# facebook/transform360

Measured on NVIDIA H100. Metric: Mpixels/s 8K equirect->cubemap bicubic (input-plane pixels consumed per second), higher is better.
Workload: dtype u8

## Files before the change

### profiles/trace_frame.py

```python
#!/usr/bin/env python
import sys
from pathlib import Path

import numpy as np
import torch

sys.path.insert(0, str(Path(__file__).resolve().parents[1]))
import transform360_b200 as t360
from bench import CONFIGS
from transform360_b200 import synth
from transform360_b200.stream import FrameTransformer, StreamSpec

KINDS = {0: "class0", 1: "class1", 3: "share-stay", 4: "share", 5: "nop", 7: "seam", 8: "pole-cap", 9: "border"}


def main():
    name = sys.argv[1] if len(sys.argv) > 1 else "cfg2"
    cfg = CONFIGS[name]
    dev = torch.device("cuda", 0)
    torch.cuda.set_device(0)
    ctx = t360.make_context(**dict(cfg["ov"], enable_low_pass_filter=0))
    spec = StreamSpec(cfg["inp"][0], cfg["inp"][1], cfg["out"][0], cfg["out"][1])
    ft = FrameTransformer(ctx, spec)
    pitch = lambda w: (w + 255) // 256 * 256
    ring = 5
    d_in = [[synth.noise_plane_torch(*spec.plane_dims(p)[:2], plane=p, frame=f, device=dev, pitch=pitch(spec.plane_dims(p)[0])) for p in range(3)]
            for f in range(ring)]
    d_out = [torch.zeros((spec.plane_dims(p)[3], pitch(spec.plane_dims(p)[2])), dtype=torch.uint8, device=dev) for p in range(3)]
    calls = [ft.frame_call([(t.data_ptr(), t.stride(0)) for t in fr], [(t.data_ptr(), t.stride(0)) for t in d_out]) for fr in d_in]
    stream = torch.cuda.Stream(device=dev)
    torch.cuda.synchronize()
    for i in range(6):
        calls[i % ring](stream.cuda_stream)
    torch.cuda.synchronize()
    ft.vft.debug_trace(True)
    calls[1](stream.cuda_stream)
    torch.cuda.synchronize()
    tr = ft.vft.read_trace().astype(np.int64)
    ft.vft.debug_trace(False)
    if len(sys.argv) > 2:
        np.save(sys.argv[2], tr)
    used = tr[..., 2] > 0
    t_start = tr[..., 0][used].min()
    end = np.where(used, tr[..., 2], 0).max(axis=1) - t_start
    begin = np.where(used, tr[..., 0], 1 << 62).min(axis=1) - t_start
    print(f"groups {tr.shape[0]}, jobs traced {int(used.sum())}, frame {end.max() / 1e3:.1f} us; groups finish at "
          f"min {end.min() / 1e3:.1f} / median {np.median(end) / 1e3:.1f} / max {end.max() / 1e3:.1f} us, start at median {np.median(begin) / 1e3:.1f} us")
    wait, comp, kind = (tr[..., 1] - tr[..., 0])[used], (tr[..., 2] - tr[..., 1])[used], tr[..., 3][used]
    print(f"all jobs: waiting {wait.sum() / 1e3:.0f} group-us, computing {comp.sum() / 1e3:.0f} group-us "
          f"({100 * wait.sum() / (wait.sum() + comp.sum()):.0f} % waiting)")
    for k in sorted(set(kind.tolist())):
        m = kind == k
        print(f"  {KINDS.get(k, k):10s} n={int(m.sum()):5d}  wait mean {wait[m].mean():7.0f} ns (p90 {np.percentile(wait[m], 90):6.0f})  "
              f"compute mean {comp[m].mean():7.0f} ns (p10 {np.percentile(comp[m], 10):6.0f} p90 {np.percentile(comp[m], 90):6.0f})")
    first = tr[:, 0, :]
    print(f"first job of a group: wait {np.mean(first[:, 1] - first[:, 0]) / 1e3:.2f} us")


if __name__ == "__main__":
    main()
```

### transform360_b200/csrc/gather_frame.cu

```cuda
#include "gather_common.cuh"

#include <cuda.h>

#include <algorithm>
#include <cstring>
#include <utility>

namespace t360 {

namespace {

template <class F, int... I>
__device__ __forceinline__ void staticForImpl(F&& f, std::integer_sequence<int, I...>) {
  (f(std::integral_constant<int, I>{}), ...);
}
template <int N, class F>
__device__ __forceinline__ void staticFor(F&& f) {
  staticForImpl(f, std::make_integer_sequence<int, N>{});
}

template <int IMM>
__device__ __forceinline__ uint32_t ldsWordImm(uint32_t addr) {
  uint32_t v;
  asm volatile("ld.shared.u32 %0, [%1+%2];" : "=r"(v) : "r"(addr), "n"(IMM));
  return v;
}
template <int IMM>
__device__ __forceinline__ uint4 ldsVecImm(uint32_t addr) {
  uint4 v;
  asm volatile("ld.shared.v4.u32 {%0, %1, %2, %3}, [%4+%5];" : "=r"(v.x), "=r"(v.y), "=r"(v.z), "=r"(v.w) : "r"(addr), "n"(IMM));
  return v;
}
template <int IMM>
__device__ __forceinline__ uint2 ldsVec2Imm(uint32_t addr) {
  uint2 v;
  asm volatile("ld.shared.v2.u32 {%0, %1}, [%2+%3];" : "=r"(v.x), "=r"(v.y) : "r"(addr), "n"(IMM));
  return v;
}

__device__ __forceinline__ uint32_t smemAddr(const void* p) { return (uint32_t)__cvta_generic_to_shared(p); }

__device__ __forceinline__ void mbarInit(uint64_t* bar, uint32_t arrivals) {
  asm volatile("mbarrier.init.shared::cta.b64 [%0], %1;" ::"r"(smemAddr(bar)), "r"(arrivals));
}
__device__ __forceinline__ void mbarExpectTx(uint64_t* bar, uint32_t bytes) {
  asm volatile("mbarrier.arrive.expect_tx.shared::cta.b64 _, [%0], %1;" ::"r"(smemAddr(bar)), "r"(bytes) : "memory");
}
__device__ __forceinline__ void mbarWait(uint64_t* bar, uint32_t parity) {
  asm volatile(
      "{\n\t.reg .pred p;\n\t"
      "WAIT_%=:\n\t"
      "mbarrier.try_wait.parity.shared::cta.b64 p, [%0], %1;\n\t"
      "@p bra DONE_%=;\n\t"
      "bra WAIT_%=;\n\t"
      "DONE_%=:\n\t}"
      ::"r"(smemAddr(bar)), "r"(parity) : "memory");
}
__device__ __forceinline__ void tmaLoadBox(void* dst, const CUtensorMap* map, int x, int y, uint64_t* bar) {
  asm volatile(
      "cp.async.bulk.tensor.2d.shared::cluster.global.mbarrier::complete_tx::bytes [%0], [%1, {%2, %3}], [%4];"
      ::"r"(smemAddr(dst)), "l"(reinterpret_cast<uint64_t>(map)), "r"(x), "r"(y), "r"(smemAddr(bar)) : "memory");
}
__device__ __forceinline__ void bulkCopyToShared(void* dst, const void* src, uint32_t bytes, uint64_t* bar) {
  asm volatile("cp.async.bulk.shared::cluster.global.mbarrier::complete_tx::bytes [%0], [%1], %2, [%3];"
               ::"r"(smemAddr(dst)), "l"(src), "r"(bytes), "r"(smemAddr(bar)) : "memory");
}
__device__ __forceinline__ void groupBarrier(int group) {
  asm volatile("bar.sync %0, %1;" ::"r"(group + 1), "n"(kGroupThreads) : "memory");
}

template <int K>
struct RowBytes {
  uint32_t b[K == 8 ? 2 : 1];
};

template <int K, int IMM>
__device__ __forceinline__ RowBytes<K> loadRow(uint32_t addr, int sh) {
  RowBytes<K> o;
  const uint32_t q0 = ldsWordImm<IMM>(addr), q1 = ldsWordImm<IMM + 4>(addr);
  o.b[0] = __funnelshift_r(q0, q1, sh);
  if constexpr (K == 8) o.b[1] = __funnelshift_r(q1, ldsWordImm<IMM + 8>(addr), sh);
  return o;
}

template <int K, int VS>
__device__ __forceinline__ int foldRows(const RowBytes<K> (&W)[K], uint32_t slotAddr) {
  int acc = 1 << 14;
  if constexpr (K == 2) {
    const uint2 w = ldsVec2Imm<0>(slotAddr);
    acc = dp2aLo(w.x, W[0].b[0], acc);
    acc = dp2aLo(w.y, W[1].b[0], acc);
  } else if constexpr (K == 4) {
    const uint4 wa = ldsVecImm<0>(slotAddr), wb = ldsVecImm<VS>(slotAddr);
    acc = dp2aLo(wa.x, W[0].b[0], acc); acc = dp2aHi(wa.y, W[0].b[0], acc);
    acc = dp2aLo(wa.z, W[1].b[0], acc); acc = dp2aHi(wa.w, W[1].b[0], acc);
    acc = dp2aLo(wb.x, W[2].b[0], acc); acc = dp2aHi(wb.y, W[2].b[0], acc);
    acc = dp2aLo(wb.z, W[3].b[0], acc); acc = dp2aHi(wb.w, W[3].b[0], acc);
  } else {
    staticFor<8>([&](auto R) {
      constexpr int r = decltype(R)::value;
      const uint4 wt = ldsVecImm<r * VS>(slotAddr);
      acc = dp2aLo(wt.x, W[r].b[0], acc); acc = dp2aHi(wt.y, W[r].b[0], acc);
      acc = dp2aLo(wt.z, W[r].b[1], acc); acc = dp2aHi(wt.w, W[r].b[1], acc);
    });
  }
  return acc;
}
template <int K>
__device__ __forceinline__ uint32_t slotOffset(uint32_t field) { return K == 2 ? field >> 1 : field; }

template <int VS>
__device__ __forceinline__ int foldRowsRotated(const RowBytes<8> (&W)[8], uint32_t wAddr, uint32_t field) {
  static_assert(VS == 16384, "one copy of the table");
  const uint32_t r = ((field >> 4) ^ threadIdx.x) & 7u;
  const uint32_t first = field ^ (r * (uint32_t)kDiagonalStep);
  const bool p0 = (r & 1u) != 0, p1 = (r & 2u) != 0, p2 = (r & 4u) != 0;
  RowBytes<8> A[8], B[8];
#pragma unroll
  for (int i = 0; i < 8; ++i)
#pragma unroll
    for (int h = 0; h < 2; ++h) A[i].b[h] = p0 ? W[i ^ 1].b[h] : W[i].b[h];
#pragma unroll
  for (int i = 0; i < 8; ++i)
#pragma unroll
    for (int h = 0; h < 2; ++h) B[i].b[h] = p1 ? A[i ^ 2].b[h] : A[i].b[h];
  int acc = 1 << 14;
  staticFor<8>([&](auto V) {
    constexpr int v = decltype(V)::value;
    const uint4 wt = ldsVecImm<0>(wAddr + (first ^ (uint32_t)(v * kDiagonalStep)));
    const uint32_t b0 = p2 ? B[v ^ 4].b[0] : B[v].b[0], b1 = p2 ? B[v ^ 4].b[1] : B[v].b[1];
    acc = dp2aLo(wt.x, b0, acc); acc = dp2aHi(wt.y, b0, acc);
    acc = dp2aLo(wt.z, b1, acc); acc = dp2aHi(wt.w, b1, acc);
  });
  return acc;
}
template <int K, int VS>
__device__ __forceinline__ int foldPixel(const RowBytes<K> (&W)[K], uint32_t wAddr, uint32_t field) {
  if constexpr (K == 8) return foldRowsRotated<VS>(W, wAddr, field);
  else return foldRows<K, VS>(W, wAddr + slotOffset<K>(field));
}
__device__ __forceinline__ int biasedToByte(int acc) { return min(max(acc >> 15, 0), 255); }


__device__ __forceinline__ uint32_t packBytes(int hi, int lo) {
  uint32_t r;
  asm("cvt.pack.sat.u8.s32.b32 %0, %1, %2, %3;" : "=r"(r) : "r"(hi), "r"(lo), "r"(0));
  return r;
}

template <int K, int PITCH, int VS, int ROWS, bool ZERO>
__device__ __forceinline__ void computeShareJob(uint8_t* dst, int dstPitch, uint32_t stageAddr, const uint4 (&rec)[ROWS / 8],
                                                uint32_t header, uint32_t wAddr) {
  static_assert(PITCH % 4 == 0 && (K == 4 || K == 8) && ROWS % 8 == 0, "");
  uint32_t base = stageAddr + (header & 0x7ffcu);
  const int sh = (int)(header << 3);
  RowBytes<K> W[K];
  staticFor<K>([&](auto R) { W[decltype(R)::value] = loadRow<K, decltype(R)::value * PITCH>(base, sh); });
  int accPrev = 0;
  staticFor<ROWS>([&](auto J) {
    constexpr int j = decltype(J)::value;
    const uint4& block = rec[j >> 3];
    const uint32_t word = ((j >> 1) & 3) == 0 ? block.x : (((j >> 1) & 3) == 1 ? block.y : (((j >> 1) & 3) == 2 ? block.z : block.w));
    const uint32_t r = (j & 1) ? word >> 16 : word;
    if constexpr (j > 0 && !ZERO) {
      const bool two = (r & 1u) != 0;
      const RowBytes<K> below = loadRow<K, (j - 1 + K) * PITCH>(base, sh);
      RowBytes<K> below2 = below;
      if (two) below2 = loadRow<K, (j + K) * PITCH>(base, sh);
#pragma unroll
      for (int q = 0; q + 2 < K; ++q)
#pragma unroll
        for (int i = 0; i < (K == 8 ? 2 : 1); ++i) W[q].b[i] = two ? W[q + 2].b[i] : W[q + 1].b[i];
#pragma unroll
      for (int i = 0; i < (K == 8 ? 2 : 1); ++i) W[K - 2].b[i] = two ? below.b[i] : W[K - 1].b[i];
      W[K - 1] = below2;
      if (two) base += PITCH;
    }
    if constexpr (j > 0 && ZERO) {
      const uint32_t d = r & 3u;
      RowBytes<K> below = W[K - 1], below2 = W[K - 1];
      if (d != 0) below = loadRow<K, K * PITCH>(base, sh);
      if (d == 2) below2 = loadRow<K, (K + 1) * PITCH>(base, sh);
#pragma unroll
      for (int q = 0; q + 2 < K; ++q)
#pragma unroll
        for (int i = 0; i < (K == 8 ? 2 : 1); ++i) W[q].b[i] = d == 0 ? W[q].b[i] : (d == 1 ? W[q + 1].b[i] : W[q + 2].b[i]);
#pragma unroll
      for (int i = 0; i < (K == 8 ? 2 : 1); ++i) {
        W[K - 2].b[i] = d == 0 ? W[K - 2].b[i] : (d == 1 ? W[K - 1].b[i] : below.b[i]);
        W[K - 1].b[i] = d == 0 ? W[K - 1].b[i] : (d == 1 ? below.b[i] : below2.b[i]);
      }
      base += d * PITCH;
    }
    const int acc = foldPixel<K, VS>(W, wAddr, r & kSlotFieldMask) >> 15;
    if constexpr (j & 1) {
      const uint32_t pair = packBytes(acc, accPrev);
      dst[(size_t)(j - 1) * dstPitch] = (uint8_t)pair;
      dst[(size_t)j * dstPitch] = (uint8_t)(pair >> 8);
    } else {
      accPrev = acc;
    }
  });
}

template <int K, int PITCH, int VS>
__device__ __forceinline__ void computeTileJob(const PlaneView& pv, uint32_t stageAddr, int outX, int outY, const uint4& rec,
                                               uint32_t wAddr, int warp) {
  static_assert(PITCH % 4 == 0, "");
  const int y0 = outY + warp * kTilePatchH;
  const int dstPitch = pv.dstPitch, dstW = pv.dstW, dstH = pv.dstH;
  uint8_t* const dstRow = pv.dst + (size_t)y0 * dstPitch + outX;
  const uint32_t words[4] = {rec.x, rec.y, rec.z, rec.w};
  staticFor<kRowsPerPatchStep>([&](auto J) {
    constexpr int j = decltype(J)::value;
    const uint32_t w = words[j];
    const int col = kTilePatchW * j + ((int)(w >> 16) & (kTilePatchW - 1)), row = (int)(w >> 19) & (kTilePatchH - 1);
    if (!(w & kRecordSkip) && outX + col < dstW && y0 + row < dstH) {
      const uint32_t rowAddr = stageAddr + (w & 0x7ffcu);
      const int sh = (int)(w << 3);
      RowBytes<K> W[K];
      staticFor<K>([&](auto R) { W[decltype(R)::value] = loadRow<K, decltype(R)::value * PITCH>(rowAddr, sh); });
      const int acc = foldPixel<K, VS>(W, wAddr, (w >> 17) & kSlotFieldMask);
      dstRow[(size_t)row * dstPitch + col] = (uint8_t)biasedToByte(acc);
    }
  });
}

template <int K, int PITCH, int VS>
__device__ __forceinline__ void computeCapJob(const PlaneView& pv, uint32_t stageAddr, uint32_t recAddr, int steps, uint32_t wAddr,
                                              int warp, int lane) {
  static_assert(PITCH % 4 == 0, "");
  for (int s = warp; s < steps; s += kGroupWarps) {
    const uint2 r = ldsVec2Imm<0>(recAddr + s * kCapStepBytes + lane * 8);
    if (r.x & kRecordSkip) continue;
    const uint32_t rowAddr = stageAddr + (r.x & 0x7ffcu);
    const int sh = (int)(r.x << 3);
    RowBytes<K> W[K];
    staticFor<K>([&](auto R) { W[decltype(R)::value] = loadRow<K, decltype(R)::value * PITCH>(rowAddr, sh); });
    const int acc = foldPixel<K, VS>(W, wAddr, (r.x >> 17) & kSlotFieldMask);
    pv.dst[(size_t)(r.y >> 16) * pv.dstPitch + (r.y & 0xffffu)] = (uint8_t)biasedToByte(acc);
  }
}

template <int K, int VS>
__device__ __forceinline__ void computeBorderJob(const PlaneView& pv, uint32_t recAddr, int n, const unsigned char* wsmem, int warp, int lane) {
  SrcView sv;
  sv.bytes = pv.src;
  sv.misalign = (int)(reinterpret_cast<uintptr_t>(pv.src) & 3);
  sv.words = reinterpret_cast<const uint32_t*>(pv.src - sv.misalign);
  sv.w = pv.srcW; sv.h = pv.srcH; sv.pitch = pv.srcPitch;
  for (int i = warp * 32 + lane; i < n; i += kGroupThreads) {
    const uint4 r = ldsVecImm<0>(recAddr + i * kBorderPixelBytes);
    const int v = gatherPixel<K, false, VS, weightDiagonal(K)>(sv, wsmem, (int)r.x, (int)r.y);
    pv.dst[(size_t)(r.z >> 16) * pv.dstPitch + (r.z & 0xffffu)] = (uint8_t)v;
  }
}

struct FrameTensorMaps {
  CUtensorMap map[kMaxFramePlanes][kNumBoxClasses][kBoxVariants];
};

__device__ __forceinline__ void mbarArrive(uint64_t* bar) {
  asm volatile("mbarrier.arrive.shared::cta.b64 _, [%0];" ::"r"(smemAddr(bar)) : "memory");
}
__device__ __forceinline__ uint4 ldsVec(uint32_t addr) {
  uint4 v;
  asm volatile("ld.shared.v4.u32 {%0, %1, %2, %3}, [%4];" : "=r"(v.x), "=r"(v.y), "=r"(v.z), "=r"(v.w) : "r"(addr));
  return v;
}
__device__ __forceinline__ uint32_t ldsWord(uint32_t addr) {
  uint32_t v;
  asm volatile("ld.shared.u32 %0, [%1];" : "=r"(v) : "r"(addr));
  return v;
}

template <int K, int COPIES, int GROUPS>
struct FrameLayout {
  static constexpr int kStages = gatherStages(K);
  static constexpr int kWeights = weightImageBytes(K, COPIES);
  static constexpr int kStage = stageBytesOf(K), kRec = stageRecordBytes(K);
  static constexpr int kGroupBytes = kStages * (kStage + kRec);
  static constexpr int kPlanes = kWeights + GROUPS * kGroupBytes;
  static constexpr int kBars = kPlanes + 256;
  static constexpr int kTotal = kBars + GROUPS * kStages * 16 + 16;
  static_assert(kTotal <= 232448, "227 KB of shared memory per CTA");
  static_assert(sizeof(PlaneView) * kMaxFramePlanes <= 256, "");
  static_assert(kStage % 128 == 0 && kRec % 128 == 0 && kWeights % 128 == 0, "TMA / bulk-copy destinations");
};

template <int K, int COPIES, int GROUPS>
__global__ void __launch_bounds__(GROUPS * (kGroupWarps + 1) * 32, 1)
gatherFrameKernel(const __grid_constant__ FrameGatherParams p, StagedParams jobs, const __grid_constant__ FrameTensorMaps maps) {
  using L = FrameLayout<K, COPIES, GROUPS>;
  constexpr int VS = weightVectorStride(K, COPIES), kStage = L::kStage, kRec = L::kRec, S = L::kStages;
  constexpr uint32_t kBox0 = stageBoxW(K, 0) * stageBoxH(K, 0), kBox1 = stageBoxW(K, 1) * stageBoxH(K, 1),
                     kBoxShare = stageBoxW(K, 2) * stageBoxH(K, 2);
  static_assert(kBox1 + 64 <= 2 * kStage && kBox0 + 64 <= kStage && kBoxShare + 64 <= kStage, "boxes must fit their stage buffers");
  static_assert(boxVariantRows(K, 0, kBoxVariants - 1) > 0 && boxVariantRows(K, 2, kBoxVariants - 1) > 0, "");
  extern __shared__ __align__(128) unsigned char smem[];
  unsigned char* wsmem = smem;
  PlaneView* planes = reinterpret_cast<PlaneView*>(smem + L::kPlanes);
  uint64_t* barBase = reinterpret_cast<uint64_t*>(smem + L::kBars);
  uint64_t* weightBar = barBase + GROUPS * 2 * S;
  const int warpId = threadIdx.x >> 5, lane = threadIdx.x & 31;
  constexpr int kProducerWarp = GROUPS * kGroupWarps;

  asm volatile("griddepcontrol.launch_dependents;" ::: "memory");
  if (threadIdx.x == 0) {
    for (int g = 0; g < GROUPS; ++g)
      for (int st = 0; st < S; ++st) {
        mbarInit(barBase + g * 2 * S + st, 1);
        mbarInit(barBase + g * 2 * S + S + st, kGroupWarps);
      }
    mbarInit(weightBar, 1);
    asm volatile("fence.mbarrier_init.release.cluster;" ::: "memory");
  }
  if (threadIdx.x < kMaxFramePlanes * (int)(sizeof(PlaneView) / 4))
    reinterpret_cast<uint32_t*>(planes)[threadIdx.x] = reinterpret_cast<const uint32_t*>(p.plane)[threadIdx.x];
  __syncthreads();

  if (warpId >= kProducerWarp) {
    const int g = warpId - kProducerWarp;
    if (g == 0 && lane == 0) {
      mbarExpectTx(weightBar, L::kWeights);
      constexpr int kChunk = L::kWeights / 4;
      for (int i = 0; i < 4; ++i)
        bulkCopyToShared(wsmem + i * kChunk, reinterpret_cast<const unsigned char*>(p.weightImage) + i * kChunk, kChunk, weightBar);
    }
    const int producer = blockIdx.x * GROUPS + g, dynamicBase = gridDim.x * GROUPS * 2 * kClaimBatch;
    auto loadBatch = [&](int base) {
      int4 h = make_int4(0, kJobExit << kJobKindShift, 0, 0);
      if (lane < kClaimBatch && base + lane < jobs.numTiles) h = __ldg(reinterpret_cast<const int4*>(jobs.tiles) + base + lane);
      return h;
    };
    int4 batch = loadBatch(producer * 2 * kClaimBatch);
    int4 batchNext = loadBatch((producer * 2 + 1) * kClaimBatch);
    asm volatile("griddepcontrol.wait;" ::: "memory");
    int claimed = 0;
    if (lane == 0) claimed = atomicAdd(jobs.claimCounter, kClaimBatch);
    unsigned char* groupBase = smem + L::kWeights + g * L::kGroupBytes;
    uint64_t* full = barBase + g * 2 * S;
    uint64_t* empty = full + S;
    int pos = 0;
    uint32_t st = 0, phase = 0;
    auto advance = [&]() { if (++st == S) { st = 0; phase ^= 1; } };
    auto postEmptyJob = [&](int kind) {
      *reinterpret_cast<int4*>(groupBase + S * kStage + st * kRec) = make_int4(0, kind << kJobKindShift, 0, 0);
      mbarArrive(full + st);
    };
    for (;;) {
      if (pos == kClaimBatch) {
        batch = batchNext;
        pos = 0;
        batchNext = loadBatch(dynamicBase + __shfl_sync(0xffffffffu, claimed, 0));
        if (lane == 0) claimed = atomicAdd(jobs.claimCounter, kClaimBatch);
      }
      int4 h;
      h.x = __shfl_sync(0xffffffffu, batch.x, pos); h.y = __shfl_sync(0xffffffffu, batch.y, pos);
      h.z = __shfl_sync(0xffffffffu, batch.z, pos); h.w = __shfl_sync(0xffffffffu, batch.w, pos);
      ++pos;
      const int kind = (h.y >> kJobKindShift) & kJobKindMask;
      mbarWait(empty + st, phase ^ 1);
      const bool twoStages = kind == kJobClass1 || kind == kJobSeam;
      if (twoStages) {
        if (st == S - 1) {
          if (lane == 0) postEmptyJob(kJobNop);
          advance();
          mbarWait(empty + st, phase ^ 1);
        }
        mbarWait(empty + st + 1, phase ^ 1);
      }
      if (lane == 0) {
        unsigned char* rec = groupBase + S * kStage + st * kRec;
        *reinterpret_cast<int4*>(rec) = h;
        if (kind == kJobExit) {
          mbarArrive(full + st);
        } else {
          const int pl = h.y >> kJobPlaneShift;
          const uint32_t recBytes = (uint32_t)jobRecordBytes(K, kind, h.x);
          if (kind == kJobBorder) {
            mbarExpectTx(full + st, recBytes);
          } else {
            const int cls = boxClassOf(kind), variant = jobBoxVariant(h.z), boxX = jobBoxX(h.z), boxY = jobBoxY(h.z);
            const uint32_t boxBytes = (uint32_t)(stageBoxW(K, cls) * boxVariantRows(K, cls, variant));
            mbarExpectTx(full + st, (kind == kJobSeam ? 2 : 1) * boxBytes + recBytes);
            tmaLoadBox(groupBase + st * kStage, &maps.map[pl][cls][variant], boxX, boxY, full + st);
            if (kind == kJobSeam)
              tmaLoadBox(groupBase + (st + 1) * kStage, &maps.map[pl][0][variant], boxX - planes[pl].srcW, boxY, full + st);
          }
          bulkCopyToShared(rec + 128, planes[pl].records + (unsigned)h.w, recBytes, full + st);
        }
      }
      advance();
      if (twoStages) {
        if (lane == 0) postEmptyJob(kJobNop);
        advance();
      }
      __syncwarp();
      if (kind == kJobExit) break;
    }
    if (lane == 0 && atomicAdd(jobs.claimCounter + 1, 1) == (int)(gridDim.x * GROUPS) - 1) {
      jobs.claimCounter[0] = 0;
      jobs.claimCounter[1] = 0;
      __threadfence();
    }
    return;
  }

  const int group = warpId / kGroupWarps, warp = warpId % kGroupWarps;
  unsigned char* groupBase = smem + L::kWeights + group * L::kGroupBytes;
  const uint32_t boxAddr = smemAddr(groupBase), recAddr = smemAddr(groupBase + S * kStage);
  uint64_t* full = barBase + group * 2 * S;
  uint64_t* empty = full + S;
  const uint32_t wAddr = smemAddr(wsmem);
  mbarWait(weightBar, 0);
  asm volatile("griddepcontrol.wait;" ::: "memory");
  auto now = []() { unsigned long long t; asm volatile("mov.u64 %0, %globaltimer;" : "=l"(t)); return t; };
  unsigned long long* trace = jobs.trace && warp == 0 && lane == 0 ? jobs.trace + (size_t)(blockIdx.x * GROUPS + group) * kTraceJobsPerGroup * 4 : nullptr;
  uint32_t traced = 0;
  for (uint32_t st = 0, phase = 0;;) {
    unsigned long long* const row = trace && traced < kTraceJobsPerGroup ? trace + traced * 4 : nullptr;
    if (row) row[0] = now();
    mbarWait(full + st, phase);
    if (row) row[1] = now();
    const uint32_t rec = recAddr + st * kRec;
    const uint4 h = ldsVec(rec);
    const int kind = ((int)h.y >> kJobKindShift) & kJobKindMask;
    if (kind == kJobExit) break;
    const int outX = (int)h.x & ~kJobQuadMask, outY = (int)h.y & kJobRowMask;
    const PlaneView& pv = planes[(int)h.y >> kJobPlaneShift];
    if (kind == kJobShare || kind == kJobShareStay) {
      if constexpr (K >= 4) {
        const uint32_t mine = rec + 128 + warp * shareWarpRecordBytes(K);
        uint4 r[shareRows(K) / 8];
#pragma unroll
        for (int b = 0; b < shareRows(K) / 8; ++b) r[b] = ldsVec(mine + b * 512 + lane * 16);
        const uint32_t header = ldsWord(mine + shareRows(K) / 8 * 512 + lane * 4);
        uint8_t* dst = pv.dst + (size_t)(outY + (warp >> 1) * shareRows(K)) * pv.dstPitch + (outX + (warp & 1) * 32 + (int)(header >> kRecordColumnShift));
        if (kind == kJobShare) computeShareJob<K, stageBoxW(K, 2), VS, shareRows(K), false>(dst, pv.dstPitch, boxAddr + st * kStage, r, header, wAddr);
        else computeShareJob<K, stageBoxW(K, 2), VS, shareRows(K), true>(dst, pv.dstPitch, boxAddr + st * kStage, r, header, wAddr);
      }
    } else if (kind == kJobClass0) {
      uint4 r;
      const int quad = ((int)h.x & kJobQuadMask) - 1;
      if (quad < 0) {
        r = ldsVec(rec + 128 + warp * 512 + lane * 16);
      } else {
        r = make_uint4(kRecordSkip, kRecordSkip, kRecordSkip, kRecordSkip);
        if ((warp >> 2) == (quad >> 1)) {
          const uint2 v = ldsVec2Imm<0>(rec + 128 + (warp & 3) * 256 + lane * 8);
          if (quad & 1) { r.z = v.x; r.w = v.y; } else { r.x = v.x; r.y = v.y; }
        }
      }
      computeTileJob<K, stageBoxW(K, 0), VS>(pv, boxAddr + st * kStage, outX, outY, r, wAddr, warp);
    } else if (kind == kJobClass1) {
      computeTileJob<K, stageBoxW(K, 1), VS>(pv, boxAddr + st * kStage, outX, outY, ldsVec(rec + 128 + warp * 512 + lane * 16), wAddr, warp);
    } else if (kind == kJobSeam) {
      {
        uint4* a = reinterpret_cast<uint4*>(groupBase + st * kStage);
        const uint4* b = reinterpret_cast<const uint4*>(groupBase + (st + 1) * kStage);
        for (int i = warp * 32 + lane; i < (int)(kBox0 / 16); i += kGroupThreads) {
          uint4 x = a[i];
          const uint4 y = b[i];
          x.x |= y.x; x.y |= y.y; x.z |= y.z; x.w |= y.w;
          a[i] = x;
        }
        asm volatile("fence.proxy.async.shared::cta;" ::: "memory");
      }
      groupBarrier(group);
      computeTileJob<K, stageBoxW(K, 0), VS>(pv, boxAddr + st * kStage, outX, outY, ldsVec(rec + 128 + warp * 512 + lane * 16), wAddr, warp);
    } else if (kind == kJobCap) {
      computeCapJob<K, stageBoxW(K, 0), VS>(pv, boxAddr + st * kStage, rec + 128, (int)h.x, wAddr, warp, lane);
    } else if (kind == kJobBorder) {
      computeBorderJob<K, VS>(pv, rec + 128, (int)h.x, wsmem, warp, lane);
    }
    __syncwarp();
    if (lane == 0) mbarArrive(empty + st);
    if (row) {
      row[2] = now(); row[3] = kind;
      ++traced;
    }
    if (++st == S) { st = 0; phase ^= 1; }
  }
}

template <int K, int COPIES, int GROUPS>
cudaError_t prepareFrameK(LaunchCfg& cfg) {
  static DeviceLaunchCfg cfgs;
  constexpr int threads = GROUPS * (kGroupWarps + 1) * 32, smemBytes = FrameLayout<K, COPIES, GROUPS>::kTotal;
  return prepare<gatherFrameKernel<K, COPIES, GROUPS>>(cfgs, threads, smemBytes, cfg);
}

template <int K, int COPIES, int GROUPS>
cudaError_t launchFrameK(const FrameGatherParams& p, const StagedParams& jobs, const FrameTensorMaps& maps, int numSMs,
                         cudaStream_t stream, bool programmatic) {
  constexpr int threads = GROUPS * (kGroupWarps + 1) * 32, smemBytes = FrameLayout<K, COPIES, GROUPS>::kTotal;
  LaunchCfg cfg;
  cudaError_t err = prepareFrameK<K, COPIES, GROUPS>(cfg);
  if (err != cudaSuccess) return err;
  const int grid = std::min(numSMs * cfg.perSM, (jobs.numTiles + GROUPS * 2 * kClaimBatch - 1) / (GROUPS * 2 * kClaimBatch));
  cudaLaunchConfig_t lc{};
  lc.gridDim = dim3(grid);
  lc.blockDim = dim3(threads);
  lc.dynamicSmemBytes = smemBytes;
  lc.stream = stream;
  cudaLaunchAttribute attr{};
  attr.id = cudaLaunchAttributeProgrammaticStreamSerialization;
  attr.val.programmaticStreamSerializationAllowed = 1;
  lc.attrs = &attr;
  lc.numAttrs = programmatic ? 1 : 0;
  err = cudaLaunchKernelEx(&lc, gatherFrameKernel<K, COPIES, GROUPS>, p, jobs, maps);
  gLaunches.fetch_add(1, std::memory_order_relaxed);
  return err;
}

}

cudaError_t prepareGatherFrame(int kernelSize) {
  LaunchCfg cfg;
  switch (kernelSize) {
    case 2: return prepareFrameK<2, weightCopies(2), gatherGroups(2)>(cfg);
    case 4: return prepareFrameK<4, weightCopies(4), gatherGroups(4)>(cfg);
    case 8: return prepareFrameK<8, weightCopies(8), gatherGroups(8)>(cfg);
    default: return cudaErrorInvalidValue;
  }
}

cudaError_t launchGatherFrame(const FrameGatherParams& p, const StagedParams& jobs, const void* tensorMaps, int numSMs,
                              cudaStream_t stream, bool programmatic) {
  if (jobs.numTiles <= 0) return cudaSuccess;
  if (p.numPlanes < 1 || p.numPlanes > kMaxFramePlanes) return cudaErrorInvalidValue;
  FrameTensorMaps maps;
  std::memcpy(&maps, tensorMaps, sizeof(CUtensorMap) * kNumBoxClasses * kBoxVariants * p.numPlanes);
  for (int i = p.numPlanes; i < kMaxFramePlanes; ++i)
    for (int c = 0; c < kNumBoxClasses; ++c)
      for (int v = 0; v < kBoxVariants; ++v) maps.map[i][c][v] = maps.map[0][c][v];
  switch (p.kernelSize) {
    case 2: return launchFrameK<2, weightCopies(2), gatherGroups(2)>(p, jobs, maps, numSMs, stream, programmatic);
    case 4: return launchFrameK<4, weightCopies(4), gatherGroups(4)>(p, jobs, maps, numSMs, stream, programmatic);
    case 8: return launchFrameK<8, weightCopies(8), gatherGroups(8)>(p, jobs, maps, numSMs, stream, programmatic);
    default: return cudaErrorInvalidValue;
  }
}

}
```

### transform360_b200/csrc/kernels.cuh

```cuda
#pragma once

#include <cuda_runtime.h>

#include <cstdint>

namespace t360 {

struct GatherParams {
  const uint8_t* src;
  int srcW, srcH, srcPitch;
  uint8_t* dst;
  int dstW, dstH, dstPitch;
  const int2* samples;
  int tilesPerRow;
  const int16_t* weights;
  int kernelSize;
  int transparent;
};

struct GatherJob {
  int outX, outY;
  int boxXY;
  int recordOffset;
};
constexpr int kBoxVariants = 3;
__host__ __device__ constexpr int jobBoxField(int boxX, int boxY, int variant) { return boxX | (boxY << 16) | variant; }
__host__ __device__ constexpr int jobBoxX(int boxXY) { return boxXY & 0xfff0; }
__host__ __device__ constexpr int jobBoxY(int boxXY) { return (int)((unsigned)boxXY >> 16); }
__host__ __device__ constexpr int jobBoxVariant(int boxXY) { return boxXY & 15; }
using StagedTile = GatherJob;
constexpr int kJobClass0 = 0, kJobClass1 = 1, kJobGeneral = 2, kJobShareStay = 3, kJobShare = 4, kJobNop = 5, kJobExit = 6, kJobSeam = 7,
              kJobCap = 8, kJobBorder = 9;
constexpr int kJobQuadMask = 7;
constexpr uint32_t kRecordSkip = 0x8000u;
constexpr int kJobKindShift = 24, kJobRowMask = (1 << kJobKindShift) - 1;
constexpr int kJobPlaneShift = 28, kJobKindMask = (1 << (kJobPlaneShift - kJobKindShift)) - 1;

constexpr int kGroupThreads = 256, kGroupWarps = kGroupThreads / 32;
__host__ __device__ constexpr int gatherGroups(int k) { return k == 8 ? 2 : 3; }
#ifndef T360_CLAIM_BATCH
#define T360_CLAIM_BATCH 1
#endif
constexpr int kClaimBatch = T360_CLAIM_BATCH;
constexpr int kGatherTileW = 32, kFrameTileH = 32;
constexpr int kTilePatchW = 8, kTilePatchH = 4, kRowsPerPatchStep = 4;
constexpr int kShareW = 64;
__host__ __device__ constexpr int shareRows(int ) { return 8; }
__host__ __device__ constexpr int shareH(int k) { return 4 * shareRows(k); }
constexpr int kNumBoxClasses = 3;
__host__ __device__ constexpr int boxClassOf(int kind) { return (kind == kJobShare || kind == kJobShareStay) ? 2 : (kind == kJobClass1 ? 1 : 0); }
__host__ __device__ constexpr int stageBoxW(int , int cls) { return cls == 2 ? 192 : (cls == 0 ? 208 : 240); }
__host__ __device__ constexpr int stageBoxH(int k, int cls) {
  return k == 8 ? (cls == 2 ? 80 : (cls == 0 ? 72 : 128)) : (cls == 2 ? 72 : (cls == 0 ? 64 : 96));
}
__host__ __device__ constexpr int boxVariantRows(int k, int cls, int v) {
  return cls == 1 || v == 0 ? stageBoxH(k, cls) : (cls == 2 ? stageBoxH(k, cls) - 8 * v : stageBoxH(k, cls) - 8 - 8 * v);
}
__host__ __device__ constexpr int boxVariantFor(int k, int cls, int rows) {
  int v = 0;
  while (v + 1 < kBoxVariants && cls != 1 && boxVariantRows(k, cls, v + 1) >= rows) ++v;
  return v;
}
__host__ __device__ constexpr int gatherStages(int ) { return 2; }
__host__ __device__ constexpr int stageBytesOf(int k) {
  const int a = stageBoxW(k, 2) * stageBoxH(k, 2), b = stageBoxW(k, 0) * stageBoxH(k, 0);
  return ((a > b ? a : b) + 64 + 127) & ~127;
}

__host__ __device__ constexpr int weightSlotOf(int k, int phase) {
  (void)k;
  return (phase & ~31) | ((phase & 1) << 4) | ((phase & 31) >> 1);
}
__host__ __device__ constexpr int weightCopies(int k) { return k == 4 ? 2 : 1; }
__host__ __device__ constexpr int weightVectorStride(int k, int copies) { return (k == 2 ? 8192 : 16384) * copies; }
__host__ __device__ constexpr int weightImageBytes(int k, int copies) { return k == 2 ? 8192 * copies : (k * k / 8) * 16384 * copies; }
__host__ __device__ constexpr int weightSlotInCopy(int slot, int copy) { return copy ? ((slot & ~7) | ((slot + copy) & 7)) : slot; }
__host__ __device__ constexpr int weightSlotField(int k, int phase, int copy) {
  return (weightSlotInCopy(weightSlotOf(k, phase), copy) << 4) | (copy << 14);
}
constexpr int kSlotFieldMask = 0x7FF0;
constexpr int kDiagonalStep = 0x4010;
__host__ __device__ constexpr bool weightDiagonal(int k) { return k == 8; }
__host__ __device__ constexpr int weightVectorOffset(int k, int copies, int slotFieldValue, int vector) {
  return weightDiagonal(k) ? (slotFieldValue ^ (vector * kDiagonalStep)) : slotFieldValue + vector * weightVectorStride(k, copies);
}
__host__ __device__ constexpr int weightBankGroups(int k) { return k == 2 ? 16 : 8; }
__host__ __device__ constexpr int weightLanesPerPass(int k) { return k == 2 ? 16 : 8; }

__host__ __device__ constexpr int shareWarpRecordBytes(int k) { return shareRows(k) / 8 * 32 * 16 + 32 * 4; }
__host__ __device__ constexpr int shareJobRecordBytes(int k) { return kGroupWarps * shareWarpRecordBytes(k); }
constexpr int kTileJobRecordBytes = kGroupWarps * 32 * 16;
constexpr int kQuadJobRecordBytes = kGroupWarps / 2 * 32 * 8;
__host__ __device__ constexpr int tileJobRecordBytes(int outXField) { return (outXField & kJobQuadMask) ? kQuadJobRecordBytes : kTileJobRecordBytes; }
__host__ __device__ constexpr int stageRecordBytes(int k) {
  return 128 + (shareJobRecordBytes(k) > kTileJobRecordBytes ? shareJobRecordBytes(k) : kTileJobRecordBytes);
}
constexpr int kCapStepBytes = 32 * 8, kBorderPixelBytes = 16;
__host__ __device__ constexpr int capJobMaxSteps(int k) { return (stageRecordBytes(k) - 128) / kCapStepBytes; }
__host__ __device__ constexpr int borderJobMaxPixels(int k) { return (stageRecordBytes(k) - 128) / kBorderPixelBytes; }
__host__ __device__ constexpr int jobRecordBytes(int k, int kind, int outXField) {
  return kind == kJobShare || kind == kJobShareStay ? shareJobRecordBytes(k)
         : kind == kJobCap                          ? outXField * kCapStepBytes
         : kind == kJobBorder                       ? outXField * kBorderPixelBytes
                                                    : tileJobRecordBytes(outXField);
}
constexpr int kRecordColumnShift = 27;

constexpr int kMaxFramePlanes = 3;
struct PlaneView {
  const uint8_t* src;
  uint8_t* dst;
  const uint4* records;
  int srcW, srcH, srcPitch;
  int dstW, dstH, dstPitch;
};
struct FrameGatherParams {
  PlaneView plane[kMaxFramePlanes];
  const uint4* weightImage;
  int kernelSize, numPlanes;
};

__host__ __device__ constexpr int gatherThreads(int k) { return k == 8 ? 512 : 256; }
__host__ __device__ constexpr int gatherTileH(int k) { return gatherThreads(k) / 32 * 4; }

struct StagedParams {
  const GatherJob* tiles;
  int numTiles;
  int* claimCounter;
  unsigned long long* trace;
};
constexpr int kTraceJobsPerGroup = 64;

struct BlurJob {
  int x0, y0, w, h;
  int kxOffset, kxCount, kyOffset, kyCount;
};

struct BlurParams {
  const uint8_t* src;
  uint8_t* dst;
  int width, height, srcPitch, dstPitch;
  const BlurJob* jobs;
  int numJobs;
  const float* taps;
  int tileSmemBytes;
};

struct StripJob {
  int x0, y0, w, h;
  int kxOffset, kxChunks, kxCount, kyOffset;
  int edge;
};

struct StripParams {
  const uint8_t* src;
  uint8_t* dst;
  int width, height, srcPitch, dstPitch;
  const StripJob* jobs;
  int numJobs;
  const float* taps;
};

struct AreaParams {
  const uint8_t* src;
  uint8_t* dst;
  int srcW, srcH, srcPitch, dstW, dstH, dstPitch;
  int cellW, cellH;
  const int2* xTaps;
  const int* xFirst;
  const int2* yTaps;
  const int* yFirst;
  const int2* xLinear;
  const int2* yLinear;
  int xMax;
};
cudaError_t launchAreaResize(const AreaParams& p, cudaStream_t stream);

struct FrameStripParams {
  struct Plane {
    const uint8_t* src;
    uint8_t* dst;
    int width, height, srcPitch, dstPitch;
  } plane[kMaxFramePlanes];
  const StripJob* jobs;
  int numJobs;
  const float* taps;
};
constexpr int kStripPlaneShift = 8;
cudaError_t launchBlurFrameStrips(const FrameStripParams& p, int hy, cudaStream_t stream);

constexpr int kStripLanePx = 8, kStripW = 32 * kStripLanePx, kStripMaxHy = 3;

constexpr int kBlurTileW = 64, kBlurTileH = 32;
constexpr int kBlurMaxSmem = 96 * 1024;

cudaError_t launchGather(const GatherParams& p, int numSMs, cudaStream_t stream);
cudaError_t launchGatherFrame(const FrameGatherParams& p, const StagedParams& jobs, const void* tensorMaps, int numSMs,
                              cudaStream_t stream, bool programmatic = true);
cudaError_t prepareGatherFrame(int kernelSize);
cudaError_t launchBlurStrips(const StripParams& p, int hy, cudaStream_t stream);
cudaError_t launchBlur(const BlurParams& p, cudaStream_t stream);
cudaError_t launchBlurDirect(const BlurParams& p, cudaStream_t stream);
unsigned long long kernelLaunchCount();
void countKernelLaunches(long long n);

inline int blurTileSmem(int w, int h, int nkx, int nky) {
  const int hx = nkx / 2, hy = nky / 2;
  const int rows = h + 2 * hy;
  const int srcStride = (w + 2 * hx + 3) & ~3;
  return rows * srcStride + rows * w * 4;
}

}
```

Before: 682,200.

## Replace fixed two-stage buffers with variable-size arena ring of job slots

The producer warp now places each job's TMA box and record into a per-group circular arena sized by the actual box variant and record length, instead of two fixed max-sized stage buffers. A six-slot descriptor ring holds header and arena offsets, and the producer waits on old slots only when the new allocation overlaps them, so more jobs can be in flight and seam jobs no longer need padding nop jobs. The claim batch also grows from one to two jobs, and the static first jobs are now single jobs. This aims to deepen prefetch and cut consumer waiting, at the cost of more complex producer bookkeeping and a risk of arena fragmentation stalls.

```diff
diff --git a/profiles/trace_frame.py b/profiles/trace_frame.py
--- a/profiles/trace_frame.py
+++ b/profiles/trace_frame.py
@@ -11,7 +11,7 @@
 from transform360_b200 import synth
 from transform360_b200.stream import FrameTransformer, StreamSpec
 
-KINDS = {0: "class0", 1: "class1", 3: "share-stay", 4: "share", 5: "nop", 7: "seam", 8: "pole-cap", 9: "border"}
+KINDS = {0: "class0", 1: "class1", 3: "share-stay", 4: "share", 7: "seam", 8: "pole-cap", 9: "border"}
 
 
 def main():
diff --git a/transform360_b200/csrc/gather_frame.cu b/transform360_b200/csrc/gather_frame.cu
--- a/transform360_b200/csrc/gather_frame.cu
+++ b/transform360_b200/csrc/gather_frame.cu
@@ -274,28 +274,46 @@
   return v;
 }
 
+__host__ __device__ constexpr int maxJobArenaBytes(int k) {
+  const int a = jobArenaBytes(2 * stageBoxW(k, 0) * stageBoxH(k, 0), kTileJobRecordBytes);
+  const int b = jobArenaBytes(stageBoxW(k, 1) * stageBoxH(k, 1), kTileJobRecordBytes);
+  const int c = jobArenaBytes((stageBoxW(k, 2) * stageBoxH(k, 2) > stageBoxW(k, 0) * stageBoxH(k, 0) ? stageBoxW(k, 2) * stageBoxH(k, 2)
+                                                                                                      : stageBoxW(k, 0) * stageBoxH(k, 0)),
+                              kJobMaxRecordBytes);
+  return a > b ? (a > c ? a : c) : (b > c ? b : c);
+}
+__host__ __device__ constexpr bool boxVariantsAligned(int k) {
+  for (int cls = 0; cls < kNumBoxClasses; ++cls)
+    for (int v = 0; v < kBoxVariants; ++v)
+      if (stageBoxW(k, cls) * boxVariantRows(k, cls, v) % 128 != 0) return false;
+  return true;
+}
+
 template <int K, int COPIES, int GROUPS>
 struct FrameLayout {
-  static constexpr int kStages = gatherStages(K);
+  static constexpr int kSmem = 232448;
+  static constexpr int kSlots = gatherRingSlots(K);
+  static constexpr int kSlotBytes = 32;
   static constexpr int kWeights = weightImageBytes(K, COPIES);
-  static constexpr int kStage = stageBytesOf(K), kRec = stageRecordBytes(K);
-  static constexpr int kGroupBytes = kStages * (kStage + kRec);
-  static constexpr int kPlanes = kWeights + GROUPS * kGroupBytes;
+  static constexpr int kFixed = kWeights + GROUPS * kSlots * kSlotBytes + 256 + GROUPS * kSlots * 16 + 16;
+  static constexpr int kArena = (kSmem - kFixed) / GROUPS / 128 * 128;
+  static constexpr int kGranule = K == 8 ? kArena / 2 / 128 * 128 : 128;
+  static constexpr int kSlotBase = kWeights + GROUPS * kArena;
+  static constexpr int kPlanes = kSlotBase + GROUPS * kSlots * kSlotBytes;
   static constexpr int kBars = kPlanes + 256;
-  static constexpr int kTotal = kBars + GROUPS * kStages * 16 + 16;
-  static_assert(kTotal <= 232448, "227 KB of shared memory per CTA");
+  static constexpr int kTotal = kBars + GROUPS * kSlots * 16 + 16;
+  static_assert(kTotal <= kSmem, "227 KB of shared memory per CTA");
   static_assert(sizeof(PlaneView) * kMaxFramePlanes <= 256, "");
-  static_assert(kStage % 128 == 0 && kRec % 128 == 0 && kWeights % 128 == 0, "TMA / bulk-copy destinations");
+  static_assert(kWeights % 128 == 0 && boxVariantsAligned(K), "TMA / bulk-copy destinations");
+  static_assert((maxJobArenaBytes(K) + kGranule - 1) / kGranule * kGranule <= kArena, "every job must fit the arena");
+  static_assert(kSlots >= 2 && kSlots <= 32, "lane i of the producer warp keeps slot i's bytes");
 };
 
 template <int K, int COPIES, int GROUPS>
 __global__ void __launch_bounds__(GROUPS * (kGroupWarps + 1) * 32, 1)
 gatherFrameKernel(const __grid_constant__ FrameGatherParams p, StagedParams jobs, const __grid_constant__ FrameTensorMaps maps) {
   using L = FrameLayout<K, COPIES, GROUPS>;
-  constexpr int VS = weightVectorStride(K, COPIES), kStage = L::kStage, kRec = L::kRec, S = L::kStages;
-  constexpr uint32_t kBox0 = stageBoxW(K, 0) * stageBoxH(K, 0), kBox1 = stageBoxW(K, 1) * stageBoxH(K, 1),
-                     kBoxShare = stageBoxW(K, 2) * stageBoxH(K, 2);
-  static_assert(kBox1 + 64 <= 2 * kStage && kBox0 + 64 <= kStage && kBoxShare + 64 <= kStage, "boxes must fit their stage buffers");
+  constexpr int VS = weightVectorStride(K, COPIES), S = L::kSlots;
   static_assert(boxVariantRows(K, 0, kBoxVariants - 1) > 0 && boxVariantRows(K, 2, kBoxVariants - 1) > 0, "");
   extern __shared__ __align__(128) unsigned char smem[];
   unsigned char* wsmem = smem;
@@ -327,32 +345,35 @@
       for (int i = 0; i < 4; ++i)
         bulkCopyToShared(wsmem + i * kChunk, reinterpret_cast<const unsigned char*>(p.weightImage) + i * kChunk, kChunk, weightBar);
     }
-    const int producer = blockIdx.x * GROUPS + g, dynamicBase = gridDim.x * GROUPS * 2 * kClaimBatch;
-    auto loadBatch = [&](int base) {
+    const int producer = blockIdx.x * GROUPS + g, dynamicBase = gridDim.x * GROUPS * 2;
+    auto loadBatch = [&](int base, int n) {
       int4 h = make_int4(0, kJobExit << kJobKindShift, 0, 0);
-      if (lane < kClaimBatch && base + lane < jobs.numTiles) h = __ldg(reinterpret_cast<const int4*>(jobs.tiles) + base + lane);
+      if (lane < n && base + lane < jobs.numTiles) h = __ldg(reinterpret_cast<const int4*>(jobs.tiles) + base + lane);
       return h;
     };
-    int4 batch = loadBatch(producer * 2 * kClaimBatch);
-    int4 batchNext = loadBatch((producer * 2 + 1) * kClaimBatch);
+    int4 batch = loadBatch(producer * 2, 1);
+    int4 batchNext = loadBatch(producer * 2 + 1, 1);
+    int size = 1, sizeNext = 1;
     asm volatile("griddepcontrol.wait;" ::: "memory");
     int claimed = 0;
     if (lane == 0) claimed = atomicAdd(jobs.claimCounter, kClaimBatch);
-    unsigned char* groupBase = smem + L::kWeights + g * L::kGroupBytes;
+    const uint32_t arena = L::kWeights + g * L::kArena;
+    unsigned char* slots = smem + L::kSlotBase + g * S * L::kSlotBytes;
     uint64_t* full = barBase + g * 2 * S;
     uint64_t* empty = full + S;
     int pos = 0;
-    uint32_t st = 0, phase = 0;
-    auto advance = [&]() { if (++st == S) { st = 0; phase ^= 1; } };
-    auto postEmptyJob = [&](int kind) {
-      *reinterpret_cast<int4*>(groupBase + S * kStage + st * kRec) = make_int4(0, kind << kJobKindShift, 0, 0);
-      mbarArrive(full + st);
-    };
+    uint32_t st = 0;
+    uint32_t old = 0, oldPhase = 0;
+    int inFlight = 0;
+    uint32_t head = 0;
+    uint32_t lo = 0, hi = 0;
     for (;;) {
-      if (pos == kClaimBatch) {
+      if (pos == size) {
         batch = batchNext;
+        size = sizeNext;
         pos = 0;
-        batchNext = loadBatch(dynamicBase + __shfl_sync(0xffffffffu, claimed, 0));
+        batchNext = loadBatch(dynamicBase + __shfl_sync(0xffffffffu, claimed, 0), kClaimBatch);
+        sizeNext = kClaimBatch;
         if (lane == 0) claimed = atomicAdd(jobs.claimCounter, kClaimBatch);
       }
       int4 h;
@@ -360,42 +381,43 @@
       h.z = __shfl_sync(0xffffffffu, batch.z, pos); h.w = __shfl_sync(0xffffffffu, batch.w, pos);
       ++pos;
       const int kind = (h.y >> kJobKindShift) & kJobKindMask;
-      mbarWait(empty + st, phase ^ 1);
-      const bool twoStages = kind == kJobClass1 || kind == kJobSeam;
-      if (twoStages) {
-        if (st == S - 1) {
-          if (lane == 0) postEmptyJob(kJobNop);
-          advance();
-          mbarWait(empty + st, phase ^ 1);
-        }
-        mbarWait(empty + st + 1, phase ^ 1);
-      }
+      const int cls = boxClassOf(kind), variant = jobBoxVariant(h.z);
+      const uint32_t boxBytes = kind == kJobExit || kind == kJobBorder ? 0u : (uint32_t)(stageBoxW(K, cls) * boxVariantRows(K, cls, variant));
+      const uint32_t recBytes = kind == kJobExit ? 0u : (uint32_t)jobRecordBytes(K, kind, h.x);
+      const uint32_t allBoxBytes = (kind == kJobSeam ? 2 : 1) * boxBytes;
+      const uint32_t need = ((uint32_t)jobArenaBytes(allBoxBytes, recBytes) + L::kGranule - 1) / L::kGranule * L::kGranule;
+      const uint32_t at = head + need <= (uint32_t)L::kArena ? head : 0u;
+      for (;;) {
+        const bool clash = lane < S && lo < at + need && at < hi;
+        if (inFlight < S && !__any_sync(0xffffffffu, clash)) break;
+        mbarWait(empty + old, oldPhase);
+        if (lane == (int)old) lo = hi = 0;
+        if (++old == S) { old = 0; oldPhase ^= 1; }
+        --inFlight;
+      }
+      if (lane == (int)st) { lo = at; hi = at + need; }
+      head = at + need;
+      ++inFlight;
       if (lane == 0) {
-        unsigned char* rec = groupBase + S * kStage + st * kRec;
-        *reinterpret_cast<int4*>(rec) = h;
+        const uint32_t box = arena + at, rec = box + (allBoxBytes ? allBoxBytes + kBoxTailBytes : 0u);
+        unsigned char* slot = slots + st * L::kSlotBytes;
+        *reinterpret_cast<int4*>(slot) = h;
+        *reinterpret_cast<uint2*>(slot + 16) = make_uint2(box, rec);
         if (kind == kJobExit) {
           mbarArrive(full + st);
         } else {
           const int pl = h.y >> kJobPlaneShift;
-          const uint32_t recBytes = (uint32_t)jobRecordBytes(K, kind, h.x);
-          if (kind == kJobBorder) {
-            mbarExpectTx(full + st, recBytes);
-          } else {
-            const int cls = boxClassOf(kind), variant = jobBoxVariant(h.z), boxX = jobBoxX(h.z), boxY = jobBoxY(h.z);
-            const uint32_t boxBytes = (uint32_t)(stageBoxW(K, cls) * boxVariantRows(K, cls, variant));
-            mbarExpectTx(full + st, (kind == kJobSeam ? 2 : 1) * boxBytes + recBytes);
-            tmaLoadBox(groupBase + st * kStage, &maps.map[pl][cls][variant], boxX, boxY, full + st);
+          mbarExpectTx(full + st, allBoxBytes + recBytes);
+          if (boxBytes) {
+            const int boxX = jobBoxX(h.z), boxY = jobBoxY(h.z);
+            tmaLoadBox(smem + box, &maps.map[pl][cls][variant], boxX, boxY, full + st);
             if (kind == kJobSeam)
-              tmaLoadBox(groupBase + (st + 1) * kStage, &maps.map[pl][0][variant], boxX - planes[pl].srcW, boxY, full + st);
+              tmaLoadBox(smem + box + boxBytes, &maps.map[pl][0][variant], boxX - planes[pl].srcW, boxY, full + st);
           }
-          bulkCopyToShared(rec + 128, planes[pl].records + (unsigned)h.w, recBytes, full + st);
+          bulkCopyToShared(smem + rec, planes[pl].records + (unsigned)h.w, recBytes, full + st);
         }
       }
-      advance();
-      if (twoStages) {
-        if (lane == 0) postEmptyJob(kJobNop);
-        advance();
-      }
+      if (++st == S) st = 0;
       __syncwarp();
       if (kind == kJobExit) break;
     }
@@ -408,8 +430,7 @@
   }
 
   const int group = warpId / kGroupWarps, warp = warpId % kGroupWarps;
-  unsigned char* groupBase = smem + L::kWeights + group * L::kGroupBytes;
-  const uint32_t boxAddr = smemAddr(groupBase), recAddr = smemAddr(groupBase + S * kStage);
+  const uint32_t smemBase = smemAddr(smem), slotAddr = smemAddr(smem + L::kSlotBase + group * S * L::kSlotBytes);
   uint64_t* full = barBase + group * 2 * S;
   uint64_t* empty = full + S;
   const uint32_t wAddr = smemAddr(wsmem);
@@ -423,43 +444,46 @@
     if (row) row[0] = now();
     mbarWait(full + st, phase);
     if (row) row[1] = now();
-    const uint32_t rec = recAddr + st * kRec;
-    const uint4 h = ldsVec(rec);
+    const uint32_t slot = slotAddr + st * L::kSlotBytes;
+    const uint4 h = ldsVec(slot);
     const int kind = ((int)h.y >> kJobKindShift) & kJobKindMask;
     if (kind == kJobExit) break;
+    const uint2 at = ldsVec2Imm<16>(slot);
+    const uint32_t box = smemBase + at.x, rec = smemBase + at.y;
     const int outX = (int)h.x & ~kJobQuadMask, outY = (int)h.y & kJobRowMask;
     const PlaneView& pv = planes[(int)h.y >> kJobPlaneShift];
     if (kind == kJobShare || kind == kJobShareStay) {
       if constexpr (K >= 4) {
-        const uint32_t mine = rec + 128 + warp * shareWarpRecordBytes(K);
+        const uint32_t mine = rec + warp * shareWarpRecordBytes(K);
         uint4 r[shareRows(K) / 8];
 #pragma unroll
         for (int b = 0; b < shareRows(K) / 8; ++b) r[b] = ldsVec(mine + b * 512 + lane * 16);
         const uint32_t header = ldsWord(mine + shareRows(K) / 8 * 512 + lane * 4);
         uint8_t* dst = pv.dst + (size_t)(outY + (warp >> 1) * shareRows(K)) * pv.dstPitch + (outX + (warp & 1) * 32 + (int)(header >> kRecordColumnShift));
-        if (kind == kJobShare) computeShareJob<K, stageBoxW(K, 2), VS, shareRows(K), false>(dst, pv.dstPitch, boxAddr + st * kStage, r, header, wAddr);
-        else computeShareJob<K, stageBoxW(K, 2), VS, shareRows(K), true>(dst, pv.dstPitch, boxAddr + st * kStage, r, header, wAddr);
+        if (kind == kJobShare) computeShareJob<K, stageBoxW(K, 2), VS, shareRows(K), false>(dst, pv.dstPitch, box, r, header, wAddr);
+        else computeShareJob<K, stageBoxW(K, 2), VS, shareRows(K), true>(dst, pv.dstPitch, box, r, header, wAddr);
       }
     } else if (kind == kJobClass0) {
       uint4 r;
       const int quad = ((int)h.x & kJobQuadMask) - 1;
       if (quad < 0) {
-        r = ldsVec(rec + 128 + warp * 512 + lane * 16);
+        r = ldsVec(rec + warp * 512 + lane * 16);
       } else {
         r = make_uint4(kRecordSkip, kRecordSkip, kRecordSkip, kRecordSkip);
         if ((warp >> 2) == (quad >> 1)) {
-          const uint2 v = ldsVec2Imm<0>(rec + 128 + (warp & 3) * 256 + lane * 8);
+          const uint2 v = ldsVec2Imm<0>(rec + (warp & 3) * 256 + lane * 8);
           if (quad & 1) { r.z = v.x; r.w = v.y; } else { r.x = v.x; r.y = v.y; }
         }
       }
-      computeTileJob<K, stageBoxW(K, 0), VS>(pv, boxAddr + st * kStage, outX, outY, r, wAddr, warp);
+      computeTileJob<K, stageBoxW(K, 0), VS>(pv, box, outX, outY, r, wAddr, warp);
     } else if (kind == kJobClass1) {
-      computeTileJob<K, stageBoxW(K, 1), VS>(pv, boxAddr + st * kStage, outX, outY, ldsVec(rec + 128 + warp * 512 + lane * 16), wAddr, warp);
+      computeTileJob<K, stageBoxW(K, 1), VS>(pv, box, outX, outY, ldsVec(rec + warp * 512 + lane * 16), wAddr, warp);
     } else if (kind == kJobSeam) {
       {
-        uint4* a = reinterpret_cast<uint4*>(groupBase + st * kStage);
-        const uint4* b = reinterpret_cast<const uint4*>(groupBase + (st + 1) * kStage);
-        for (int i = warp * 32 + lane; i < (int)(kBox0 / 16); i += kGroupThreads) {
+        const int n = stageBoxW(K, 0) * boxVariantRows(K, 0, jobBoxVariant((int)h.z)) / 16;
+        uint4* a = reinterpret_cast<uint4*>(smem + at.x);
+        const uint4* b = a + n;
+        for (int i = warp * 32 + lane; i < n; i += kGroupThreads) {
           uint4 x = a[i];
           const uint4 y = b[i];
           x.x |= y.x; x.y |= y.y; x.z |= y.z; x.w |= y.w;
@@ -468,11 +492,11 @@
         asm volatile("fence.proxy.async.shared::cta;" ::: "memory");
       }
       groupBarrier(group);
-      computeTileJob<K, stageBoxW(K, 0), VS>(pv, boxAddr + st * kStage, outX, outY, ldsVec(rec + 128 + warp * 512 + lane * 16), wAddr, warp);
+      computeTileJob<K, stageBoxW(K, 0), VS>(pv, box, outX, outY, ldsVec(rec + warp * 512 + lane * 16), wAddr, warp);
     } else if (kind == kJobCap) {
-      computeCapJob<K, stageBoxW(K, 0), VS>(pv, boxAddr + st * kStage, rec + 128, (int)h.x, wAddr, warp, lane);
+      computeCapJob<K, stageBoxW(K, 0), VS>(pv, box, rec, (int)h.x, wAddr, warp, lane);
     } else if (kind == kJobBorder) {
-      computeBorderJob<K, VS>(pv, rec + 128, (int)h.x, wsmem, warp, lane);
+      computeBorderJob<K, VS>(pv, rec, (int)h.x, wsmem, warp, lane);
     }
     __syncwarp();
     if (lane == 0) mbarArrive(empty + st);
@@ -498,7 +522,7 @@
   LaunchCfg cfg;
   cudaError_t err = prepareFrameK<K, COPIES, GROUPS>(cfg);
   if (err != cudaSuccess) return err;
-  const int grid = std::min(numSMs * cfg.perSM, (jobs.numTiles + GROUPS * 2 * kClaimBatch - 1) / (GROUPS * 2 * kClaimBatch));
+  const int grid = std::min(numSMs * cfg.perSM, (jobs.numTiles + GROUPS * 2 - 1) / (GROUPS * 2));
   cudaLaunchConfig_t lc{};
   lc.gridDim = dim3(grid);
   lc.blockDim = dim3(threads);
diff --git a/transform360_b200/csrc/kernels.cuh b/transform360_b200/csrc/kernels.cuh
--- a/transform360_b200/csrc/kernels.cuh
+++ b/transform360_b200/csrc/kernels.cuh
@@ -29,7 +29,7 @@
 __host__ __device__ constexpr int jobBoxY(int boxXY) { return (int)((unsigned)boxXY >> 16); }
 __host__ __device__ constexpr int jobBoxVariant(int boxXY) { return boxXY & 15; }
 using StagedTile = GatherJob;
-constexpr int kJobClass0 = 0, kJobClass1 = 1, kJobGeneral = 2, kJobShareStay = 3, kJobShare = 4, kJobNop = 5, kJobExit = 6, kJobSeam = 7,
+constexpr int kJobClass0 = 0, kJobClass1 = 1, kJobGeneral = 2, kJobShareStay = 3, kJobShare = 4, kJobExit = 6, kJobSeam = 7,
               kJobCap = 8, kJobBorder = 9;
 constexpr int kJobQuadMask = 7;
 constexpr uint32_t kRecordSkip = 0x8000u;
@@ -39,7 +39,7 @@
 constexpr int kGroupThreads = 256, kGroupWarps = kGroupThreads / 32;
 __host__ __device__ constexpr int gatherGroups(int k) { return k == 8 ? 2 : 3; }
 #ifndef T360_CLAIM_BATCH
-#define T360_CLAIM_BATCH 1
+#define T360_CLAIM_BATCH 2
 #endif
 constexpr int kClaimBatch = T360_CLAIM_BATCH;
 constexpr int kGatherTileW = 32, kFrameTileH = 32;
@@ -61,11 +61,9 @@
   while (v + 1 < kBoxVariants && cls != 1 && boxVariantRows(k, cls, v + 1) >= rows) ++v;
   return v;
 }
-__host__ __device__ constexpr int gatherStages(int ) { return 2; }
-__host__ __device__ constexpr int stageBytesOf(int k) {
-  const int a = stageBoxW(k, 2) * stageBoxH(k, 2), b = stageBoxW(k, 0) * stageBoxH(k, 0);
-  return ((a > b ? a : b) + 64 + 127) & ~127;
-}
+__host__ __device__ constexpr int gatherRingSlots(int ) { return 6; }
+constexpr int kBoxTailBytes = 128;
+__host__ __device__ constexpr int jobArenaBytes(int boxBytes, int recBytes) { return ((boxBytes ? boxBytes + kBoxTailBytes : 0) + recBytes + 127) & ~127; }
 
 __host__ __device__ constexpr int weightSlotOf(int k, int phase) {
   (void)k;
@@ -92,12 +90,11 @@
 constexpr int kTileJobRecordBytes = kGroupWarps * 32 * 16;
 constexpr int kQuadJobRecordBytes = kGroupWarps / 2 * 32 * 8;
 __host__ __device__ constexpr int tileJobRecordBytes(int outXField) { return (outXField & kJobQuadMask) ? kQuadJobRecordBytes : kTileJobRecordBytes; }
-__host__ __device__ constexpr int stageRecordBytes(int k) {
-  return 128 + (shareJobRecordBytes(k) > kTileJobRecordBytes ? shareJobRecordBytes(k) : kTileJobRecordBytes);
-}
+constexpr int kJobMaxRecordBytes = 5120;
+static_assert(shareJobRecordBytes(4) <= kJobMaxRecordBytes && shareJobRecordBytes(8) <= kJobMaxRecordBytes && kTileJobRecordBytes <= kJobMaxRecordBytes, "");
 constexpr int kCapStepBytes = 32 * 8, kBorderPixelBytes = 16;
-__host__ __device__ constexpr int capJobMaxSteps(int k) { return (stageRecordBytes(k) - 128) / kCapStepBytes; }
-__host__ __device__ constexpr int borderJobMaxPixels(int k) { return (stageRecordBytes(k) - 128) / kBorderPixelBytes; }
+__host__ __device__ constexpr int capJobMaxSteps(int ) { return kJobMaxRecordBytes / kCapStepBytes; }
+__host__ __device__ constexpr int borderJobMaxPixels(int ) { return kJobMaxRecordBytes / kBorderPixelBytes; }
 __host__ __device__ constexpr int jobRecordBytes(int k, int kind, int outXField) {
   return kind == kJobShare || kind == kJobShareStay ? shareJobRecordBytes(k)
          : kind == kJobCap                          ? outXField * kCapStepBytes
```

Result: faster. 696,200, median of 6 (+2.1%).
